# mehta-lab/VisCy

Hardware: AMD Instinct MI355X
Metric: training patches/sec (Z=5, 256x256, 1->2ch UNeXt2) (higher is better)
Workload: dtype bf16; 1 GPU; UNeXt2 2.5D convnextv2_tiny Z=5 256x256 1->2ch, fwd+MixedLoss(0.5,0,0.5)+bwd+AdamW; per_gpu_batch=512, global_batch=512, parallelism=dp1

## Files before the change

viscy_amd/csrc/gemm.hip:

```cpp
#include "vsx_common.h"
#include "mfma16.h"
#include "../../include/vsx.h"

bool vsx_gemm_nt2_ok(const VsxGemm* p);
bool vsx_gemm_nt2_lnbwd_ok(const VsxGemm* p);
void vsx_gemm_nt2_plan(const VsxGemm* p, VsxGemmPlan& pl);
int vsx_gemm_nt2_run(const VsxGemmPlan& pl, const VsxGemm* p, hipStream_t s);

struct RowCoord {
  int b, y, x;
  bool valid;
};

__device__ __forceinline__ RowCoord decode_row(const VsxGemm& p, int m) {
  RowCoord r;
  r.valid = m < p.M;
  int mm = r.valid ? m : 0;
  if (p.a_mode == VSX_A_ROWS && p.c_mode == VSX_A_ROWS) {
    r.b = p.hw > 0 ? mm / p.hw : 0;
    r.y = 0;
    r.x = mm;
  } else {
    int hw = p.gh * p.gw;
    r.b = mm / hw;
// ... 1092 lines not shown
#pragma unroll
    for (int i = 0; i < NCHX; ++i)
      if (livex[i]) xr[i] = ldvec_stream<T>(reinterpret_cast<const T*>(Xs + xoff[i]), x_once);
#pragma unroll
    for (int i = 0; i < NCHY; ++i)
      if (livey[i]) yr[i] = ldvec_stream<T>(reinterpret_cast<const T*>(Ys + yoff[i]), y_once);
  };
  float gsr[VN], gbr[VN];
  int gcur = -1;
  if constexpr (PRO == 1) {
#pragma unroll
    for (int j = 0; j < VN; ++j) gbr[j] = p.grn_b[kcol[0] + j];
  }
  auto store_tiles = [&](int step, int buf, const vec* xr, const vec* yr) {
    char* Xs = smem + buf * (TILE_X + TILE_Y);
    char* Ys = Xs + TILE_X;
    if constexpr (PRO == 1) {
      const int bnow = (step * BMS) / p.hw;
      if (bnow != gcur) {
        gcur = bnow;
        const float* gs = p.grn_s + (size_t)bnow * p.K + kcol[0];
#pragma unroll
        for (int j = 0; j < VN; ++j) gsr[j] = gs[j];
      }
    }
#pragma unroll
    for (int i = 0; i < NCHX; ++i) {
      if (livex[i]) {
        const vec xv = xr[i];
        *reinterpret_cast<vec*>(Xs + ldsx[i]) = xv;
      }
    }
#pragma unroll
    for (int i = 0; i < NCHY; ++i) {
      if (livey[i]) {
        vec yv = yr[i];
        if constexpr (PRO == 1) {
          float f[VN];
          unpack<T>(yv, f);
#pragma unroll
          for (int j = 0; j < VN; ++j) f[j] = fmaf(f[j], gsr[j], gbr[j]);
          yv = pack<T>(f);
        }
        *reinterpret_cast<vec*>(Ys + ldsy[i]) = yv;
      }
    }
  };

  mf_f32x4 acc[FN_][FK_];
  mfma_zero(acc);
  float csum = 0.f;
  const bool do_colsum = p.colsum != nullptr && tile_k == 0 && tid < BTN;
  mf_f32x4 acc2[PRO == 2 ? FN_ : 1][PRO == 2 ? FK_ : 1];
  float sreg[PRO == 2 ? FK_ : 1];
  mf_f32x4 acc1[2] = {{0.f, 0.f, 0.f, 0.f}, {0.f, 0.f, 0.f, 0.f}};
  frag_t ones_frag;
  const bool want_p = PRO == 2 && p.aux != nullptr && p.red0 != nullptr;
  if constexpr (PRO == 2) {
    union { unsigned short h[8]; frag_t v; } one;
#pragma unroll
    for (int j = 0; j < 8; ++j) one.h[j] = 0x3F80;
    ones_frag = one.v;
    mfma_zero(acc2);
    if (want_p) {
      const unsigned short* W2 = reinterpret_cast<const unsigned short*>(p.aux);
#pragma unroll
      for (int i = 0; i < FN_; ++i)
#pragma unroll
        for (int j = 0; j < FK_; ++j) {
          const int k = k0 + (wk * FK_ + j) * 16 + p16;
          unsigned short w[4];
#pragma unroll
          for (int r = 0; r < 4; ++r) {
            const int n = n0 + (wn * FN_ + i) * 16 + kq * 4 + r;
            w[r] = (n < p.N && k < p.K) ? W2[(size_t)n * p.ldx + k] : (unsigned short)0;
          }
          w2img[(i * FK_ + j) * 256 + tid] = make_uint2((uint32_t)w[0] | ((uint32_t)w[1] << 16), (uint32_t)w[2] | ((uint32_t)w[3] << 16));
        }
    }
  }

  const bool contig = (p.pro & 1024) != 0;
  const int sps = PRO == 2 ? p.hw / BMS : 1;
  const int units = total_steps / sps;
  const int sq = units / nsplit, sr = units % nsplit;
  const int sbase = (by * sq + (by < sr ? by : sr)) * sps;
  const int nsteps = contig ? (sq + (by < sr ? 1 : 0)) * sps : (total_steps - by + nsplit - 1) / nsplit;
  auto step_of = [&](int st) { return contig ? sbase + st : st * nsplit + by; };
  auto mma_step = [&](const char* Xs, const char* Ys) {
#pragma unroll
    for (int kk = 0; kk < BMS / MK; ++kk) {
      const char* Xk = Xs + (sizeof(T) == 2 ? kk * 32 * LDBX : 0);
      const char* Yk = Ys + (sizeof(T) == 2 ? kk * 32 * LDBY : 0);
      constexpr int JH = FK_ > 8 ? 2 : 1, JW = FK_ / JH;
      static_assert(FK_ % JH == 0, "Y fragments split evenly");
      frag_t xf[FN_], yf[JW];
#pragma unroll
      for (int i = 0; i < FN_; ++i) xf[i] = lds_frag_mn<T, TR>(Xk, LDBX, (wn * FN_ + i) * 16, p16, kq, kk);
#pragma unroll
      for (int jh = 0; jh < JH; ++jh) {
#pragma unroll
        for (int j = 0; j < JW; ++j) yf[j] = lds_frag_mn<T, TR>(Yk, LDBY, (wk * FK_ + jh * JW + j) * 16, p16, kq, kk);
#pragma unroll
        for (int i = 0; i < FN_; ++i)
#pragma unroll
          for (int j = 0; j < JW; ++j) acc[i][jh * JW + j] = mfma16(xf[i], yf[j], acc[i][jh * JW + j]);
      }
      if constexpr (PRO == 2) {
        static_assert(PRO != 2 || FN_ == 4, "two X fragments per wave");
#pragma unroll
        for (int h = 0; h < 2; ++h) acc1[h] = mfma16(wk == 0 ? xf[h] : xf[2 + h], ones_frag, acc1[h]);
      }
    }
    if constexpr (PRO == 2) {
    } else if (do_colsum) {
#pragma unroll 8
      for (int r = 0; r < BMS; ++r) csum += to_f32<T>(*reinterpret_cast<const T*>(Xs + r * LDBX + tid * ES));
    }
  };
  auto sample_begin = [&](int gstep) {
    if constexpr (PRO == 2) {
      const float* gs = p.grn_s + (size_t)(gstep / sps) * p.K;
#pragma unroll
      for (int j = 0; j < FK_; ++j) {
        const int k = k0 + (wk * FK_ + j) * 16 + p16;
        sreg[j] = gs[k < p.K ? k : p.K - 1];
      }
    }
  };
  auto sample_end = [&](int gstep) {
    if constexpr (PRO == 2) {
      if (want_p) {
        float pj[FK_];
#pragma unroll
        for (int j = 0; j < FK_; ++j) {
          float a = 0.f;
#pragma unroll
          for (int i = 0; i < FN_; ++i) {
            const uint2 w = w2img[(i * FK_ + j) * 256 + tid];
            a = fmaf(acc[i][j][0], __uint_as_float(w.x << 16), a);
            a = fmaf(acc[i][j][1], __uint_as_float(w.x & 0xFFFF0000u), a);
            a = fmaf(acc[i][j][2], __uint_as_float(w.y << 16), a);
            a = fmaf(acc[i][j][3], __uint_as_float(w.y & 0xFFFF0000u), a);
          }
          a += __shfl_xor(a, 16, 64);
          a += __shfl_xor(a, 32, 64);
          pj[j] = a;
        }
        if (kq == 0) {
          float* P = p.red0 + (size_t)(gstep / sps) * p.K;
#pragma unroll
          for (int j = 0; j < FK_; ++j) {
            const int k = k0 + (wk * FK_ + j) * 16 + p16;
            if (k < p.K) atomicAdd(P + k, pj[j]);
          }
        }
      }
#pragma unroll
      for (int i = 0; i < FN_; ++i)
#pragma unroll
        for (int j = 0; j < FK_; ++j)
#pragma unroll
          for (int r = 0; r < 4; ++r) {
            acc2[i][j][r] = fmaf(acc[i][j][r], sreg[j], acc2[i][j][r]);
            acc[i][j][r] = 0.f;
          }
    }
  };
  load_tiles(step_of(0), xreg, yreg);
  if constexpr (NBUF == 2) {
    store_tiles(step_of(0), 0, xreg, yreg);
    __syncthreads();
    for (int st = 0; st < nsteps; ++st) {
      const int nxt = step_of(st + 1);
      if (st + 1 < nsteps) load_tiles(nxt, xreg, yreg);
      const char* Xs = smem + (st & 1) * (TILE_X + TILE_Y);
      mma_step(Xs, Xs + TILE_X);
      if (st + 1 < nsteps) store_tiles(nxt, (st + 1) & 1, xreg, yreg);
      __syncthreads();
    }
  } else {
    static_assert(PRO != 2 || NBUF == 1, "the post-scaled weight gradient lives on the single-buffer geometry");
    for (int st = 0; st < nsteps; ++st) {
      store_tiles(step_of(st), 0, xreg, yreg);
      __syncthreads();
      if (st + 1 < nsteps) load_tiles(step_of(st + 1), xreg, yreg);
      if constexpr (PRO == 2) {
        if ((sbase + st) % sps == 0) sample_begin(sbase + st);
      }
      mma_step(smem, smem + TILE_X);
      if constexpr (PRO == 2) {
        if ((sbase + st + 1) % sps == 0) sample_end(sbase + st);
      }
      __syncthreads();
    }
  }
  if constexpr (PRO == 2) {
    float* cs = reinterpret_cast<float*>(smem);
    __syncthreads();
    if (p16 == 0) {
#pragma unroll
      for (int h = 0; h < 2; ++h)
#pragma unroll
        for (int r = 0; r < 4; ++r) cs[(wn * FN_ + 2 * wk + h) * 16 + kq * 4 + r] = acc1[h][r];
    }
    __syncthreads();
    if (tid < BTN) csum = cs[tid];
#pragma unroll
    for (int j = 0; j < FK_; ++j) {
      const int k = k0 + (wk * FK_ + j) * 16 + p16;
      const float bk = p.grn_b[k < p.K ? k : p.K - 1];
#pragma unroll
      for (int i = 0; i < FN_; ++i)
#pragma unroll
        for (int r = 0; r < 4; ++r) acc[i][j][r] = fmaf(bk, cs[(wn * FN_ + i) * 16 + kq * 4 + r], acc2[i][j][r]);
    }
  }

  const bool per_sample = p.b_bstride != 0;
  const bool ps_atomic = (p.pro & 4096) != 0;
  const int sample = per_sample ? (int)(((long)sbase * BMS) / p.hw) : 0;
  float* W = reinterpret_cast<float*>(p.C) + p.c_coff[z] + (per_sample ? (size_t)sample * (size_t)p.b_bstride : 0);
#pragma unroll
  for (int i = 0; i < FN_; ++i)
#pragma unroll
    for (int j = 0; j < FK_; ++j)
#pragma unroll
      for (int r = 0; r < 4; ++r) {
        const int n = n0 + (wn * FN_ + i) * 16 + kq * 4 + r;
        const int k = k0 + (wk * FK_ + j) * 16 + p16;
        if (n < p.N && k < p.K) {
          if (per_sample && !ps_atomic) W[(size_t)n * p.ldc + k] = acc[i][j][r];
          else atomicAdd(W + (size_t)n * p.ldc + k, acc[i][j][r]);
        }
      }
  if (do_colsum && n0 + tid < p.N) {
    if (per_sample && !ps_atomic) p.colsum[(size_t)sample * p.N + n0 + tid] = csum;
    else atomicAdd(p.colsum + (per_sample ? (size_t)sample * p.N : 0) + n0 + tid, csum);
  }
}

__global__ __launch_bounds__(256) void tn_zero_kernel(float* __restrict__ p, long n) {
  long i = ((long)blockIdx.x * 256 + threadIdx.x) * 4;
  if (i + 3 < n) *reinterpret_cast<float4*>(p + i) = make_float4(0.f, 0.f, 0.f, 0.f);
  else for (; i < n; ++i) p[i] = 0.f;
}

static double last_round_fill(long wgs, int per_cu) {
  const long slots = 256 * per_cu, rounds = (wgs + slots - 1) / slots;
  return (double)wgs / (double)(rounds * slots);
}

static int fill_splits(int tiles, int per_cu, int want, int max_splits) {
  if (!g_vsx_tn_fill) return want;
  int lo = want * 2 / 3, hi = want * 4 / 3;
  lo = lo < 1 ? 1 : lo;
  hi = hi > max_splits ? max_splits : hi;
  int best = want < lo ? lo : (want > hi ? hi : want);
  double best_fill = -1.0;
  for (int sp = lo; sp <= hi; ++sp) {
    const double fill = last_round_fill((long)tiles * sp, per_cu);
    const int d = sp > want ? sp - want : want - sp, bd = best > want ? best - want : want - best;
    if (fill > best_fill + 1e-9 || (fill > best_fill - 1e-9 && d < bd)) { best_fill = fill; best = sp; }
  }
  return best;
}

static int fill_sample_splits(int tiles, int per_cu, int ks, int steps) {
  if (!g_vsx_tn_fill) return ks;
  int best = ks;
  double best_fill = -1.0;
  for (int sp = ks; sp <= 4 * ks && sp <= 64 && steps % sp == 0; sp *= 2) {
    const double fill = last_round_fill((long)tiles * sp, per_cu);
    if (fill > best_fill + 1e-9) { best_fill = fill; best = sp; }
  }
  return best;
}

static int plan_tn(const VsxGemm* p, int dtype, VsxGemmPlan& pl) {
  if (int e = check_common(p, dtype, "vsx_gemm_tn")) return e;
  VSX_CHECK(p->epi == VSX_EPI_NONE && p->c_mode == VSX_A_ROWS, "vsx_gemm_tn: no epilogue / scatter modes");
  const long t128 = (long)vsx_cdiv(p->N, 128) * vsx_cdiv(p->K, 128);
  bool small = (p->N < 96 || p->K < 96) || (t128 < 24 && p->M < 65536);
  if (p->b_bstride != 0) small = false;
  const bool stats = p->pro == VSX_PRO_GRN && p->aux != nullptr && p->red0 != nullptr;
  if (stats) {
    VSX_CHECK(dtype == VSX_BF16 && g_vsx_tn_tr, "vsx_gemm_tn: the weight gradient with GRN statistics (aux = W2, red0 = P) is a bf16 kernel");
    small = false;
  }
  const int es = dtype == VSX_BF16 ? 2 : 4, vn = 16 / es, BT = small ? 64 : 128, nz = p->nz > 0 ? p->nz : 1;
  const bool TR = es == 2 && g_vsx_tn_tr, lean128 = TR && BT == 128;
  const unsigned long long ld_bytes = (unsigned long long)(p->lda > p->ldb ? p->lda : p->ldb) * es;
  const int stream_bits = (g_vsx_tn_stream & 3) << 13;
  pl = VsxGemmPlan{};
  pl.family = FAM_TN_FAST;
  pl.esize = es; pl.tr = TR; pl.tile[0] = pl.tile[1] = BT; pl.step = 32; pl.nbuf = 2; pl.block = 256;
  const int tiles = vsx_cdiv(p->N, BT) * vsx_cdiv(p->K, BT);
  const int want = vsx_cdiv(g_vsx_tn_want, tiles * nz), max_splits = vsx_cdiv(p->M, 256);
  int splits = want < 1 ? 1 : (want > max_splits ? max_splits : want);
  const int cap = tiles * nz <= 4 ? 384 : (tiles * nz <= 24 ? 96 : 48);
  if (splits > cap) splits = cap;
  if (splits > vsx_cdiv(p->M, 32)) splits = vsx_cdiv(p->M, 32);
  if (splits >= 8) splits &= ~7;
  pl.grid[0] = tiles; pl.grid[1] = splits; pl.grid[2] = nz;
  if (p->b_bstride != 0) {
    VSX_CHECK(lean128, "vsx_gemm_tn: per-sample outputs (b_bstride) exist for bf16 operands with outputs of at least 96 x 96 only");
    VSX_CHECK((g_vsx_nt_fast & 1) && p->a_mode == VSX_A_ROWS && p->pro == VSX_PRO_NONE && p->hw > 0 && p->hw % 64 == 0 && p->M % p->hw == 0 &&
                  nz == 1 && 64 * ld_bytes < (1ull << 31),
              "vsx_gemm_tn: per-sample outputs (b_bstride) need plain bf16 row operands, no prologue, hw %% 64 == 0");
    const int nb = p->M / p->hw;
    const bool n_full = p->N >= 192 && p->N <= 256 && p->K >= 128;
    const int t2 = n_full ? vsx_cdiv(p->N, 256) * vsx_cdiv(p->K, 128) : tiles;
    int ks = 1;
    const int spp = p->hw / 64;
    while ((long)nb * ks * t2 < 768 && ks < 64 && spp % (2 * ks) == 0) ks *= 2;
    if (ks > 1) ks = fill_sample_splits(nb * t2, n_full ? 2 : 3, ks, spp);
    pl.pro_bits = 1024 | stream_bits;
    if (ks > 1) {
      pl.pro_bits |= 4096;
      pl.zero_c = (long)nb * p->b_bstride;
      pl.zero_colsum = p->colsum ? (long)nb * p->N : 0;
    }
    if (n_full) { pl.tile[0] = 256; pl.tile[1] = 128; }
    pl.step = 64; pl.nbuf = 1;
    pl.grid[0] = t2; pl.grid[1] = nb * ks;
    return 0;
  }
  if (stats) {
    VSX_CHECK((g_vsx_nt_fast & 1) && p->a_mode == VSX_A_ROWS && nz == 1 && p->hw > 0 && p->hw % 64 == 0 && p->M % p->hw == 0 && p->N >= 96 &&
                  p->K >= 128 && p->N % 8 == 0 && p->K % 8 == 0 && p->ldx >= p->K && 64 * ld_bytes < (1ull << 31),
              "vsx_gemm_tn: the weight gradient with GRN statistics (aux = W2, red0 = P) needs plain bf16 row operands, hw %% 64 == 0, N >= 96, K >= 128");
    const int nb = p->M / p->hw;
    int sp = 1;
    if (g_vsx_tn_p2_rounds > 0) {
      sp = (g_vsx_tn_p2_rounds * 512) / tiles;
    } else {
      const int wantp = vsx_cdiv(g_vsx_tn_want * 2, tiles);
      for (int d = wantp < nb ? wantp : nb; d >= 1; --d)
        if (nb % d == 0) { sp = d; break; }
    }
    pl.pro_kind = 2; pl.step = 64; pl.nbuf = 1;
    pl.pro_bits = 1024 | stream_bits;
    pl.grid[1] = sp < 1 ? 1 : (sp > nb ? nb : sp);
    return 0;
  }
  const bool patch_ok = (g_vsx_nt_fast & 2) && p->a_mode == VSX_A_PATCH2 && p->pro == VSX_PRO_NONE && p->gw > 0 && (32 % p->gw == 0 || p->gw % 64 == 0) &&
                        p->cs % vn == 0 && (unsigned long long)(512 + 4 * p->gw) * p->lda * es < (1ull << 31);
  const bool fast = (g_vsx_nt_fast & 1) && (p->a_mode == VSX_A_ROWS || patch_ok) && p->M % 32 == 0 && p->N >= vn && p->K >= vn &&
                    (p->pro == VSX_PRO_NONE || (p->pro == VSX_PRO_GRN && p->hw > 0 && p->hw % 32 == 0)) && 32 * ld_bytes < (1ull << 31);
  if (!fast) {
    pl.family = FAM_TN_GEN;
    pl.step = pl.nbuf = 0;
    return 0;
  }
  pl.pro_kind = p->pro == VSX_PRO_GRN;
  pl.pro_bits = (g_vsx_tn_contig ? 1024 : 0) | stream_bits;
  if (!(es == 2 && BT == 128 && g_vsx_tn_wide && p->M % 64 == 0 && (p->pro == VSX_PRO_NONE || p->hw % 64 == 0) && p->M / 64 >= 2 * splits))
    return 0;
  pl.step = 64; pl.nbuf = 1;
  if (!TR) return 0;
  if (g_vsx_tn_fill) {
    int spf = fill_splits(tiles * nz, 3, splits, p->M / 128);
    if (spf > cap) spf = cap;
    pl.grid[1] = spf < 1 ? 1 : spf;
  }
  const bool n_div = (g_vsx_tn_rect & 2) && p->N % 256 == 0 && p->K >= 128 && p->pro == VSX_PRO_NONE;
  const bool n_full = ((g_vsx_tn_rect & 1) && p->N >= 224 && p->N <= 256 && p->K >= 256) || n_div;
  const bool k_full = (g_vsx_tn_rect & 1) && !n_full && p->K >= 224 && p->K <= 256 && p->N >= 256;
  if (!n_full && !k_full) return 0;
  pl.tile[0] = n_full ? 256 : 128; pl.tile[1] = n_full ? 128 : 256;
  const int t2 = vsx_cdiv(p->N, pl.tile[0]) * vsx_cdiv(p->K, pl.tile[1]);
  const int want2 = vsx_cdiv(g_vsx_tn_want2, t2 * nz);
  int sp2 = want2 < 1 ? 1 : (want2 > max_splits ? max_splits : want2);
  if (sp2 > p->M / 128) sp2 = p->M / 128;
  if (g_vsx_tn_fill) sp2 = fill_splits(t2 * nz, 2, sp2, p->M / 128);
  else if (sp2 >= 8) sp2 &= ~7;
  pl.grid[0] = t2; pl.grid[1] = sp2 < 1 ? 1 : sp2;
  return 0;
}

static int run_tn(const VsxGemmPlan& pl, const VsxGemm* p, hipStream_t s) {
  VsxGemm q = *p;
  q.pro = (pl.pro_kind == 2 ? 0 : q.pro) | pl.pro_bits;
  if (pl.zero_c) hipLaunchKernelGGL(tn_zero_kernel, dim3(vsx_cdiv(pl.zero_c, 1024L)), dim3(256), 0, s, reinterpret_cast<float*>(p->C) + p->c_coff[0], (long)pl.zero_c);
  if (pl.zero_colsum) hipLaunchKernelGGL(tn_zero_kernel, dim3(vsx_cdiv(pl.zero_colsum, 1024L)), dim3(256), 0, s, p->colsum, (long)pl.zero_colsum);
  const dim3 grid(pl.grid[0], pl.grid[1], pl.grid[2]), block(pl.block);
#define TN_GEN(T, BT, TR) \
  case inst_key(true, sizeof(T), BT, BT, 0, 0, 0, TR, 0): hipLaunchKernelGGL((gemm_tn_kernel<T, BT, TR>), grid, block, 0, s, q, 0); break;
#define TN_FAST1(T, BT, TR, PRO, BMS, NBUF, BTK) \
  case inst_key(false, sizeof(T), BT, BTK ? BTK : BT, BMS, NBUF, PRO, TR, 0): hipLaunchKernelGGL((gemm_tn_fast_kernel<T, BT, TR, PRO, BMS, NBUF, BTK>), grid, block, 0, s, q); break;
#define TN_FAST(T, BT, TR, BMS, NBUF, BTK)  TN_FAST1(T, BT, TR, 0, BMS, NBUF, BTK) TN_FAST1(T, BT, TR, 1, BMS, NBUF, BTK)
  switch (inst_key(pl)) {
    TN_GEN(bf16_t, 64, true) TN_GEN(bf16_t, 128, true) TN_GEN(bf16_t, 64, false) TN_GEN(bf16_t, 128, false) TN_GEN(float, 64, false) TN_GEN(float, 128, false)
    TN_FAST(bf16_t, 64, true, 32, 2, 0) TN_FAST(bf16_t, 128, true, 32, 2, 0)
    TN_FAST(bf16_t, 64, false, 32, 2, 0) TN_FAST(bf16_t, 128, false, 32, 2, 0)
    TN_FAST(float, 64, false, 32, 2, 0) TN_FAST(float, 128, false, 32, 2, 0)
    TN_FAST(bf16_t, 128, true, 64, 1, 0) TN_FAST(bf16_t, 128, false, 64, 1, 0)
    TN_FAST(bf16_t, 256, true, 64, 1, 128)
    TN_FAST(bf16_t, 128, true, 64, 1, 256)
    TN_FAST1(bf16_t, 128, true, 2, 64, 1, 0)
    default: vsx_set_error("vsx_gemm_tn: the plan names no instantiation"); return 1;
  }
#undef TN_GEN
#undef TN_FAST1
#undef TN_FAST
  VSX_LAUNCH_CHECK();
  g_vsx_last_kernel = pl.family;
  return 0;
}

extern "C" int32_t vsx_gemm_tn(const VsxGemm* p, int32_t dtype, vsx_stream_t stream) {
  VsxGemmPlan pl;
  if (int e = plan_tn(p, dtype, pl)) return e;
  return run_tn(pl, p, reinterpret_cast<hipStream_t>(stream));
}

extern "C" int32_t vsx_gemm_plan(int32_t kind, const VsxGemm* p, int32_t dtype, VsxGemmPlan* out) {
  VSX_CHECK(out != nullptr && (kind == VSX_GEMM_NT || kind == VSX_GEMM_TN), "vsx_gemm_plan: kind %d, out %p", kind, (void*)out);
  return kind == VSX_GEMM_NT ? plan_nt(p, dtype, *out) : plan_tn(p, dtype, *out);
}
```

viscy_amd/engine_unext2.py:

```python

from __future__ import annotations

import os
from collections import namedtuple
from typing import NamedTuple

import torch
from torch import Tensor

from . import _lib as L
from . import ops as hip_ops
from .flat import FlatEngine, engine_apply


class _BlockW:

    __slots__ = ("C", "p", "dw_w", "W1f", "W1fT", "b1f", "W2", "W2T", "v1", "fc2_w", "fc2_b", "grn_w", "grn_b", "dp", "img", "img2", "b2f")


class _ProjW:
    __slots__ = ("cin", "cout", "taps", "ln", "conv", "W", "WT")


FWD_UNFUSED, FWD_PAIR, FWD_FC1 = 0, 1, 2


class _MlpPlan(NamedTuple):

    fwd: int
    ln_in: bool
    keep_h: bool
    keep_xh: bool
    bwd: int
    tn_stats: bool


def _plan_mlp(flag: int, supported, C: int, hw: int, M: int, B: int, dt: torch.dtype, training: bool, ln_bwd_ok: bool,
              tn_stats_ok: bool) -> _MlpPlan:
    if dt != torch.bfloat16:
        flag = 0
    if not training:
        pair = bool(flag & 1) and supported(None)
        return _MlpPlan(FWD_PAIR if pair else FWD_UNFUSED, pair and bool(flag & 32), False, False, 0, False)
    fc1 = bool(flag & 2) and supported(2)
    bwd = 0
    if flag & 8 and supported(4):
        if B * C * 4 * C * 4 <= (512 << 20) and C >= 96 and hw % 64 == 0:
            bwd = 1
        elif supported(3):
            bwd = 2
    recompute_h = bool(flag & 64) and bwd != 0 and supported(5) and supported(6)
    drop_xh = bool(flag & 128) and bool(flag & 32) and recompute_h and supported(7) and ln_bwd_ok
    ln_in = fc1 and bool(flag & 32)
    return _MlpPlan(FWD_FC1 if fc1 else FWD_UNFUSED, ln_in, not (fc1 and recompute_h), not (ln_in and drop_xh), bwd,
                    bwd == 2 and bool(tn_stats_ok))


_BlockSaved = namedtuple("_BlockSaved", "x xh rstd h gact colsq s rows dpm plan y mean")
_NarrowSaved = namedtuple("_NarrowSaved", "x y colsq s")


def _views(flat: Tensor, shapes):
    out, off = [], 0
    for shp in shapes:
        n = 1
        for s in shp:
            n *= s
        out.append(flat[off : off + n].view(shp))
        off += n
    return out


class _ZeroArena:

    def __init__(self, dev, numel: int, ops):
        self.dev, self.ops = dev, ops
        self.buf = self._zeros(numel) if numel > 0 else None
        self.off = 0
        self.used = 0

    def _zeros(self, *shape) -> Tensor:
        return self.ops.zeros(*shape, device=self.dev)

    def take(self, *shape) -> Tensor:
        n = 1
        for d in shape:
            n *= int(d)
        n_al = (n + 63) // 64 * 64
        self.used += n_al
        if self.buf is not None and self.off + n_al <= self.buf.numel():
            v = self.buf[self.off:self.off + n].view(*shape)
            self.off += n_al
            return v
        return self._zeros(*shape)


class Engine(FlatEngine):
    name = "UNeXt2"

    def __init__(self, model, ops=None):
        ops = hip_ops if ops is None else ops
        self._hip = ops is hip_ops
        self._mlp_flag = 0
        self.cfg = model.cfg
        self._zeros4c = {}
        self._dp_inject = None
        self._za = None
        self._za_need = {}
        self._prepared_for = None
        self.W = None
        super().__init__(model, ops)

    def _stage_params_rev(self, stage):
        ps = []
        for blk in reversed(list(stage.blocks)):
            if hasattr(blk, "gamma"):
                ps += [blk.gamma, blk.mlp.fc2.weight, blk.mlp.fc2.bias, blk.mlp.fc1.weight, blk.mlp.fc1.bias, blk.norm.weight,
                       blk.norm.bias, blk.conv_dw.weight, blk.conv_dw.bias]
                continue
            ps += [blk.mlp.fc2.weight, blk.mlp.fc2.bias, blk.mlp.grn.weight, blk.mlp.grn.bias, blk.mlp.fc1.weight,
                   blk.mlp.fc1.bias, blk.norm.weight, blk.norm.bias, blk.conv_dw.weight, blk.conv_dw.bias]
        if not isinstance(stage.downsample, torch.nn.Identity):
            ps += [stage.downsample[1].weight, stage.downsample[1].bias, stage.downsample[0].weight,
                   stage.downsample[0].bias]
        return ps

    def _param_order(self):
        m = self.model
        ps = []
        if self.cfg.get("head", "conv") == "conv":
# ... 100 lines not shown
        narrow_stem = cfg.get("head") == "shuffle" and tuple(cfg["stem_kernel"][1:]) == (2, 2)
        if narrow_stem and K % 8 and Dp == 1:
            W["stem_W"], W["stem_b"] = None, m.stem.conv.bias
        elif Dp == 1:
            W["stem_W"], _ = o.prep_weight(sw, co3, K, 1, dt)
            if dt == torch.bfloat16 and K % 32:
                o.flush()
                W["stem_W"] = o.pad_cols(W["stem_W"], (K + 31) // 32 * 32)
            W["stem_b"] = m.stem.conv.bias
        else:
            we = torch.zeros((co3, Dp, Dp, K), dtype=torch.float32, device=self.device)
            for d in range(Dp):
                we[:, d, d, :] = sw.detach().reshape(co3, K)
            W["stem_W"] = we.reshape(co3 * Dp, Dp * K).to(dt).contiguous()
            W["stem_b"] = m.stem.conv.bias.detach().repeat_interleave(Dp).contiguous()
        s2 = getattr(m, "stem2d", None)
        if s2 is not None:
            K2 = s2.weight[0].numel()
            W["stem2d_W"] = None
            if not (narrow_stem and K2 % 8):
                W["stem2d_W"], _ = o.prep_weight(s2.weight, s2.weight.shape[0], K2, 1, dt)
            if W["stem2d_W"] is not None and dt == torch.bfloat16 and K2 % 32:
                o.flush()
                W["stem2d_W"] = o.pad_cols(W["stem2d_W"], (K2 + 31) // 32 * 32)
            W["stem2d_b"] = s2.bias
        enc = []
        for i in range(4):
            st = getattr(m.encoder_stages, f"stages_{i}")
            proj = None
            if not isinstance(st.downsample, torch.nn.Identity):
                proj = self._prep_proj(st.downsample[0], st.downsample[1], dt, need_bwd)
            enc.append((proj, [self._prep_block(b, dt, need_bwd) for b in st.blocks]))
        rates = cfg.get("drop_path")
        if rates:
            flat_blocks = [bw for _, blocks in enc for bw in blocks]
            assert len(rates) == len(flat_blocks)
            for bw, r in zip(flat_blocks, rates):
                bw.dp = float(r)
        W["enc"] = enc
        dec = []
        if cfg.get("head") == "embed":
            t = m.tail
            E, Cf = t.fc0.weight.shape
            P = t.fc3.weight.shape[0]
            W["fc0"], W["fc0T"] = o.prep_weight(t.fc0.weight, E, Cf, 1, torch.float32, want=True, want_t=need_bwd)
            W["fc3"], W["fc3T"] = o.prep_weight(t.fc3.weight, P, E, 1, torch.float32, want=True, want_t=need_bwd)
        else:
            for us in m.decoder.decoder_stages:
                st = us.conv
                proj = self._prep_proj(st.downsample[0], st.downsample[1], dt, need_bwd)
                dec.append((proj, [self._prep_block(b, dt, need_bwd) for b in st.blocks]))
            pre = []
            for us in m.decoder.decoder_stages:
                pc = getattr(us, "pre_conv", None)
                if pc is None:
                    pre.append(None)
                else:
                    cpc = pc.weight.shape[0]
                    pre.append((pc, *o.prep_weight(pc.weight, cpc, cpc, 9, dt, want=True, want_t=need_bwd)))
            W["dec_pre"] = pre
        W["dec"] = dec
        if cfg.get("head", "conv") == "conv":
            hc = m.head.conv[0].conv
            cmid, c3 = hc.weight.shape[0], hc.weight.shape[1]
            hdt = self._head_dtype(dt)
            W["head_Wc"], _ = o.prep_weight(hc.weight, cmid, c3, 27, hdt, tapmode=1)
            if need_bwd:
                if hdt == torch.bfloat16 and c3 == 8 and cmid == 32 and cfg["out_stack_depth"] == 5:
                    o.flush()
                    W["head_Wp"] = o.head_conv_dgrad_prep(W["head_Wc"])
                W["head_Wd"] = o.prep_head_dgrad(hc.weight, cmid, c3, cfg["out_stack_depth"], hdt)
        return W

    def _head_dtype(self, dt: torch.dtype) -> torch.dtype:
        if dt == torch.bfloat16 and self.model.head.conv[0].conv.weight.shape[1] % 8:
            return torch.float32
        return dt

    def _plan(self, C, hw, M, B, dt, training: bool) -> _MlpPlan:
        o, flag = self.ops, self._mlp_flag
        ask = training and dt == torch.bfloat16 and flag != 0
        return _plan_mlp(flag, lambda mode: o.mlp_supported(C, hw, M, dt, mode), C, hw, M, B, dt, training,
                         ask and bool(L.lib().vsx_gemm_nt_ln_bwd_supported(M, C, 4 * C, L.dtype_code(dt))),
                         ask and o.tn_grn_stats_ok(M, C, 4 * C, hw, dt))

    def _block_fwd(self, x, w, B, H, Wd, dt, save, rows=None):
        if w.C < 16:
            return self._block_fwd_narrow(x, w, B, H, Wd, save, rows)
        o = self.ops
        C, M = w.C, B * H * Wd
        blk = w.p
        hw = H * Wd
        y = o.dwconv7_fwd(x, w.dw_w, blk.conv_dw.bias, B, H, Wd, C)
        xres = x
        if rows is not None:
            idx, inv, _, Lr = rows
            M, hw = B * Lr, Lr
            y = o.rows_select(y, idx, M, C)
            xres = o.rows_select(x, idx, M, C)
        plan = self._plan(C, hw, M, B, dt, save is not None)
        mean = rstd = None
        if plan.ln_in:
            xh = None
        else:
            xh, _, rstd = o.ln_fwd(y, None, None, M, C, 1e-6, need_mean=False)
            y = None
        colsq = self._za.take(B, 4 * C)
        dpm = None
        if w.dp > 0.0 and self.model.training:
            inj = self._dp_inject
            dpm = inj.pop(0) if inj else (torch.rand(B, device=x.device) < (1.0 - w.dp)).float() / (1.0 - w.dp)
        assert plan.fwd == FWD_UNFUSED or w.img is not None
        if plan.fwd == FWD_PAIR:
            src, lne = (y, 1e-6) if plan.ln_in else (xh, 0.0)
            o.mlp_stats(src, w.img, w.b1f, colsq, M, C, hw, ln_eps=lne)
            s = o.grn_scale(colsq, w.grn_w)
            out = o.mlp_out(src, w.img, w.b1f, s, w.grn_b, w.fc2_b, xres, dpm, M, C, hw, ln_eps=lne)
            if rows is not None:
                out = o.rows_select(out, rows[1], B * H * Wd, C)
            return out
        if plan.fwd == FWD_FC1:
            if plan.ln_in:
                first, rstd, h, gact = o.mlp_fc1_ln(y, w.img, w.b1f, colsq, M, C, hw, 1e-6, store_h=plan.keep_h,
                                                    store_xh=plan.keep_xh)
                xh, y, mean = (first, None, None) if plan.keep_xh else (None, *first)
                del first
            else:
                h, gact = o.mlp_fc1(xh, w.img, w.b1f, colsq, M, C, hw, store_h=plan.keep_h)
        else:
            h = torch.empty((M, 4 * C), dtype=dt, device=x.device) if save is not None else None
            gact = torch.empty((M, 4 * C), dtype=dt, device=x.device)
            o.gemm("nt", xh, w.W1f, h, M, 4 * C, C, C, C, 4 * C, dtype=dt, epi=L.EPI_BIAS_GELU_SQ, bias=w.b1f, red0=colsq,
                   hw=hw, C2=gact)
        s = o.grn_scale(colsq, w.grn_w)
        out = torch.empty((M, C), dtype=dt, device=x.device)
        if dt == torch.bfloat16 and C > 64 and hw % 128 == 0 and hw // 128 >= 8:
            Ws = o.scale_weight_samples(w.fc2_w, s, dt)
            b2 = w.b2f
            if b2 is None:
                b2 = o.matvec(w.fc2_w, w.grn_b, w.fc2_b, C, 4 * C)
                o.flush()
            o.gemm("nt", gact, Ws, out, M, C, 4 * C, 4 * C, 4 * C, C, dtype=dt, hw=hw, b_bstride=C * 4 * C,
                   epi=L.EPI_BIAS_RES, bias=b2, res=xres, ldr=C, rscale=dpm)
        else:
            o.gemm("nt", gact, w.W2, out, M, C, 4 * C, 4 * C, 4 * C, C, dtype=dt, pro=L.PRO_GRN, grn_s=s,
                   grn_b=w.grn_b, hw=hw, epi=L.EPI_BIAS_RES, bias=w.fc2_b, res=xres, ldr=C, rscale=dpm)
        if rows is not None:
            out = o.rows_select(out, rows[1], B * H * Wd, C)
        if save is not None:
            save.append(_BlockSaved(x, xh, rstd, h, gact, colsq, s, rows, dpm, plan, y, mean))
        return out

    def _block_fwd_narrow(self, x, w, B, H, Wd, save, rows):
        o, C = self.ops, w.C
        if rows is not None or w.v1 or (w.dp > 0.0 and self.model.training):
            raise NotImplementedError("narrow ConvNeXt blocks are built for dense ConvNeXt-V2 decoder stages only")
        colsq = self._za.take(B, 4 * C)
        y = o.narrow_block_fwd1(x, w.dw_w, w.p.conv_dw.bias, w.W1f, w.b1f, colsq, B, H, Wd, C)
        s = o.grn_scale(colsq, w.grn_w)
        out = o.narrow_block_fwd2(y, x, w.W1f, w.b1f, s, w.grn_b, w.W2, w.fc2_b, B, H, Wd, C)
        if save is not None:
            save.append(_NarrowSaved(x, y, colsq, s))
        return out

    def _block_bwd_narrow(self, dout, w, saved, B, H, Wd):
        o, g = self.ops, self.g
        C, blk = w.C, w.p
# ... 485 lines not shown
```

viscy_amd/ops.py:

```python

from __future__ import annotations

import contextlib
import ctypes as C
import os
import threading
from typing import Sequence

import torch
from torch import Tensor

from . import _lib as L
from ._lib import VsxGemm, VsxGemmPlan, check, dtype_code, lib, ptr, stream


class Scratch:

    def __init__(self, alloc=None):
        self._alloc = alloc or (lambda floats, dev: torch.empty(floats, dtype=torch.float32, device=dev))
        self._tls = threading.local()
        self.held: list = []

    def take(self, dev, floats: int):
        arenas = getattr(self._tls, "arenas", None)
# ... 39 lines not shown
        for i, v in enumerate(vals):
            arr[i] = int(v)


def gemm(
    kind: str,
    A: Tensor,
    B: Tensor,
    Cout: Tensor,
    M: int,
    N: int,
    K: int,
    lda: int,
    ldb: int,
    ldc: int,
    *,
    dtype: torch.dtype,
    a_mode: int = L.A_ROWS,
    gh: int = 0,
    gw: int = 0,
    cs: int = 0,
    nz: int = 1,
    a_coff: Sequence[int] | None = None,
    b_off: Sequence[int] | None = None,
    c_coff: Sequence[int] | None = None,
    c_mode: int = L.A_ROWS,
    c_cs: int = 0,
    pro: int = L.PRO_NONE,
    grn_s: Tensor | None = None,
    grn_b: Tensor | None = None,
    hw: int = 0,
    epi: int = L.EPI_NONE,
    bias: Tensor | None = None,
    res: Tensor | None = None,
    ldr: int = 0,
    aux: Tensor | None = None,
    ldx: int = 0,
    red0: Tensor | None = None,
    red1: Tensor | None = None,
    colsum: Tensor | None = None,
    C2: Tensor | None = None,
    b_bstride: int = 0,
    rscale: Tensor | None = None,
    plan: VsxGemmPlan | None = None,
) -> None:
    for t in (bias, grn_s, grn_b, red0, red1, colsum):
        if t is not None and t.dtype != torch.float32:
            raise TypeError("bias / GRN / reduction buffers must be float32")
    p = VsxGemm()
    p.A, p.B, p.C = ptr(A), ptr(B), ptr(Cout)
    p.M, p.N, p.K = M, N, K
    p.lda, p.ldb, p.ldc = lda, ldb, ldc
    p.a_mode, p.gh, p.gw, p.cs = a_mode, gh, gw, cs
    p.nz = nz
    _fill8(p.a_coff, a_coff)
    _fill8(p.b_off, b_off)
    _fill8(p.c_coff, c_coff)
    p.c_mode, p.c_cs = c_mode, c_cs
    p.pro = pro
    p.grn_s, p.grn_b = ptr(grn_s), ptr(grn_b)
    p.hw = hw
    p.epi = epi
    p.bias, p.res, p.ldr = ptr(bias), ptr(res), ldr
    p.aux, p.ldx = ptr(aux), ldx
    p.red0, p.red1, p.colsum = ptr(red0), ptr(red1), ptr(colsum)
    p.C2 = ptr(C2)
    p.b_bstride = b_bstride
    p.rscale = ptr(rscale)
    if plan is not None:
        return check(lib().vsx_gemm_plan(L.GEMM_NT if kind == "nt" else L.GEMM_TN, C.byref(p), dtype_code(dtype), C.byref(plan)), f"gemm_plan_{kind}")
    if kind == "nt" and epi == L.EPI_BIAS_GELU_SQ:
        _det(A.device, lambda: _gemm_det_floats(p, dtype))
    fn = lib().vsx_gemm_nt if kind == "nt" else lib().vsx_gemm_tn
    check(fn(C.byref(p), dtype_code(dtype), stream()), f"gemm_{kind}")


def _gemm_det_floats(p: VsxGemm, dtype: torch.dtype) -> int:
    plan = VsxGemmPlan()
    check(lib().vsx_gemm_plan(L.GEMM_NT, C.byref(p), dtype_code(dtype), C.byref(plan)), "gemm_plan_nt")
    return plan.det_floats


def tn_grn_stats_ok(M: int, N: int, K: int, hw: int, dtype: torch.dtype) -> bool:
    if dtype != torch.bfloat16 or not lib().vsx_get_flag(b"tn_rect") & 8:
        return False
    p = VsxGemm()
    p.A = p.B = p.C = p.grn_s = p.grn_b = p.aux = p.red0 = 1
    p.M, p.N, p.K, p.lda, p.ldb, p.ldc, p.ldx, p.nz, p.pro, p.hw = M, N, K, K, N, K, K, 1, L.PRO_GRN, hw
    return lib().vsx_gemm_plan(L.GEMM_TN, C.byref(p), L.VSX_BF16, C.byref(VsxGemmPlan())) == 0


def dgrad_ln_bwd(dh: Tensor, WT: Tensor, xh: Tensor, rstd: Tensor, M: int, C: int, K: int,
                 mean: Tensor | None = None) -> Tensor | None:
    if dh.dtype != torch.bfloat16 or not lib().vsx_gemm_nt_ln_bwd_supported(M, C, K, dtype_code(dh.dtype)):
        return None
    dy = torch.empty((M, C), dtype=dh.dtype, device=dh.device)
    gemm("nt", dh, WT, dy, M, C, K, K, K, C, dtype=dh.dtype, epi=L.EPI_LN_BWD, aux=xh, ldx=C, grn_s=rstd, grn_b=mean)
    return dy


def gemm_z(kind: str, *args, nz: int, a_coff, b_off, c_coff, **kw) -> None:
    for s in range(0, nz, 8):
        e = min(nz, s + 8)
        gemm(kind, *args, nz=e - s, a_coff=a_coff[s:e], b_off=b_off[s:e], c_coff=c_coff[s:e], **kw)


def ln_fwd(x: Tensor, gamma: Tensor | None, beta: Tensor | None, rows: int, Cc: int, eps: float = 1e-6,
           need_mean: bool = True):
    y = torch.empty_like(x)
    mean = torch.empty(rows, dtype=torch.float32, device=x.device) if need_mean else None
    rstd = torch.empty(rows, dtype=torch.float32, device=x.device)
    check(lib().vsx_ln_fwd(ptr(x), ptr(y), ptr(mean), ptr(rstd), ptr(gamma), ptr(beta), rows, Cc, eps,
                           dtype_code(x.dtype), stream()), "ln_fwd")
    return y, mean, rstd


def ln_bwd(dy: Tensor, x: Tensor, mean: Tensor | None, rstd: Tensor, gamma: Tensor | None, add: Tensor | None,
           dgamma: Tensor | None, dbeta: Tensor | None, rows: int, Cc: int) -> Tensor:
    dx = torch.empty_like(dy)
    check(lib().vsx_ln_bwd(ptr(dy), ptr(x), ptr(mean), ptr(rstd), ptr(gamma), ptr(add), ptr(dx), ptr(dgamma),
                           ptr(dbeta), rows, Cc, dtype_code(dy.dtype), stream()), "ln_bwd")
    return dx


def grn_scale(colsq: Tensor, gamma: Tensor, eps: float = 1e-6) -> Tensor:
    s = torch.empty_like(colsq)
    check(lib().vsx_grn_scale(ptr(colsq), ptr(gamma), ptr(s), colsq.shape[0], colsq.shape[1], eps, stream()), "grn_scale")
    return s


def grn_bwd_stats(colsq: Tensor, P: Tensor, gamma: Tensor, dgamma: Tensor, eps: float = 1e-6, Sb: Tensor | None = None,
                  dbeta: Tensor | None = None) -> Tensor:
    t = torch.empty_like(colsq)
    rowst = torch.empty_like(colsq)
    if _BATCH is not None:
        nb, N = colsq.shape
        check(lib().vsx_grn_bwd_stats(ptr(colsq), ptr(P), None, ptr(gamma), ptr(t), None, None, ptr(rowst), nb, N, eps, stream()),
              "grn_bwd_stats")
        _queue(L.WTASK_REDUCE_ROWS, 0, (nb, N), rowst, dgamma, None, None)
        if Sb is not None:
            _queue(L.WTASK_REDUCE_ROWS, 0, (nb, N), Sb, dbeta, None, None)
        return t
    check(lib().vsx_grn_bwd_stats(ptr(colsq), ptr(P), ptr(Sb), ptr(gamma), ptr(t), ptr(dgamma), ptr(dbeta), ptr(rowst), colsq.shape[0],
                                  colsq.shape[1], eps, stream()), "grn_bwd_stats")
    return t


def grn_gelu_bwd(dz: Tensor, h: Tensor, s: Tensor, t: Tensor, colsum: Tensor, M: int, N: int, hw: int) -> None:
    rows = 2048
    ws = _workspace(dz.device, rows * N)
    check(lib().vsx_grn_gelu_bwd(ptr(dz), ptr(h), ptr(s), ptr(t), ptr(colsum), ptr(ws), rows, M, N, hw,
                                 dtype_code(dz.dtype), stream()), "grn_gelu_bwd")


def dwconv7_fwd(x: Tensor, w: Tensor, bias: Tensor | None, B: int, H: int, W: int, Cc: int) -> Tensor:
    y = torch.empty_like(x)
    check(lib().vsx_dwconv7_fwd(ptr(x), ptr(w), ptr(bias), None, ptr(y), B, H, W, Cc, dtype_code(x.dtype), stream()),
          "dwconv7_fwd")
    return y


def dwconv7_bwd_data(dy: Tensor, w: Tensor, add: Tensor | None, B: int, H: int, W: int, Cc: int) -> Tensor:
    dx = torch.empty_like(dy)
    check(lib().vsx_dwconv7_bwd_data(ptr(dy), ptr(w), ptr(add), ptr(dx), B, H, W, Cc, dtype_code(dy.dtype), stream()),
          "dwconv7_bwd_data")
    return dx


def dwconv7_bwd_weight(dy: Tensor, x: Tensor, dw: Tensor, db: Tensor | None, B: int, H: int, W: int, Cc: int) -> None:
    rows = 256
    ws = _workspace(dy.device, rows * 50 * Cc)
    check(lib().vsx_dwconv7_bwd_weight(ptr(dy), ptr(x), ptr(dw), ptr(db), ptr(ws), rows, B, H, W, Cc, dtype_code(dy.dtype),
# ... 1184 lines not shown
```

Measured before the change: 5637 patches/s.

## Allow sub-sample step splits in GRN-stats weight-gradient GEMM and prefer it when grid fills

The GRN-statistics weight-gradient kernel can now split work at step granularity instead of whole-sample units when there are too few samples per split, with partial samples accumulating their P contributions through the existing atomics. The planner accepts a negative rounds flag that sets the split count directly, above the sample count. The MLP planner selects the fused stats backward (bwd=2) for C<=192 when the resulting grid has at least 384 blocks. The P dot product also accumulates in a 4-wide vector FMA. This trades more atomic traffic for better GPU occupancy on narrow stages.

```diff
diff --git a/viscy_amd/csrc/gemm.hip b/viscy_amd/csrc/gemm.hip
--- a/viscy_amd/csrc/gemm.hip
+++ b/viscy_amd/csrc/gemm.hip
@@ -1198,10 +1198,11 @@
 
   const bool contig = (p.pro & 1024) != 0;
   const int sps = PRO == 2 ? p.hw / BMS : 1;
-  const int units = total_steps / sps;
+  const int unit = total_steps / sps >= 8 * nsplit ? sps : 1;
+  const int units = total_steps / unit;
   const int sq = units / nsplit, sr = units % nsplit;
-  const int sbase = (by * sq + (by < sr ? by : sr)) * sps;
-  const int nsteps = contig ? (sq + (by < sr ? 1 : 0)) * sps : (total_steps - by + nsplit - 1) / nsplit;
+  const int sbase = (by * sq + (by < sr ? by : sr)) * unit;
+  const int nsteps = contig ? (sq + (by < sr ? 1 : 0)) * unit : (total_steps - by + nsplit - 1) / nsplit;
   auto step_of = [&](int st) { return contig ? sbase + st : st * nsplit + by; };
   auto mma_step = [&](const char* Xs, const char* Ys) {
 #pragma unroll
@@ -1250,15 +1251,15 @@
         float pj[FK_];
 #pragma unroll
         for (int j = 0; j < FK_; ++j) {
-          float a = 0.f;
+          mf_f32x4 a4 = {0.f, 0.f, 0.f, 0.f};
 #pragma unroll
           for (int i = 0; i < FN_; ++i) {
             const uint2 w = w2img[(i * FK_ + j) * 256 + tid];
-            a = fmaf(acc[i][j][0], __uint_as_float(w.x << 16), a);
-            a = fmaf(acc[i][j][1], __uint_as_float(w.x & 0xFFFF0000u), a);
-            a = fmaf(acc[i][j][2], __uint_as_float(w.y << 16), a);
-            a = fmaf(acc[i][j][3], __uint_as_float(w.y & 0xFFFF0000u), a);
+            const mf_f32x4 wf = {__uint_as_float(w.x << 16), __uint_as_float(w.x & 0xFFFF0000u), __uint_as_float(w.y << 16),
+                                 __uint_as_float(w.y & 0xFFFF0000u)};
+            a4 = __builtin_elementwise_fma(acc[i][j], wf, a4);
           }
+          float a = (a4[0] + a4[1]) + (a4[2] + a4[3]);
           a += __shfl_xor(a, 16, 64);
           a += __shfl_xor(a, 32, 64);
           pj[j] = a;
@@ -1302,11 +1303,11 @@
       __syncthreads();
       if (st + 1 < nsteps) load_tiles(step_of(st + 1), xreg, yreg);
       if constexpr (PRO == 2) {
-        if ((sbase + st) % sps == 0) sample_begin(sbase + st);
+        if (st == 0 || (sbase + st) % sps == 0) sample_begin(sbase + st);
       }
       mma_step(smem, smem + TILE_X);
       if constexpr (PRO == 2) {
-        if ((sbase + st + 1) % sps == 0) sample_end(sbase + st);
+        if (st + 1 == nsteps || (sbase + st + 1) % sps == 0) sample_end(sbase + st);
       }
       __syncthreads();
     }
@@ -1447,8 +1448,11 @@
                   p->K >= 128 && p->N % 8 == 0 && p->K % 8 == 0 && p->ldx >= p->K && 64 * ld_bytes < (1ull << 31),
               "vsx_gemm_tn: the weight gradient with GRN statistics (aux = W2, red0 = P) needs plain bf16 row operands, hw %% 64 == 0, N >= 96, K >= 128");
     const int nb = p->M / p->hw;
-    int sp = 1;
-    if (g_vsx_tn_p2_rounds > 0) {
+    int sp = 1, max_sp = nb;
+    if (g_vsx_tn_p2_rounds < 0) {
+      sp = -g_vsx_tn_p2_rounds;
+      max_sp = p->M / 64 < 65535 ? p->M / 64 : 65535;
+    } else if (g_vsx_tn_p2_rounds > 0) {
       sp = (g_vsx_tn_p2_rounds * 512) / tiles;
     } else {
       const int wantp = vsx_cdiv(g_vsx_tn_want * 2, tiles);
@@ -1457,7 +1461,7 @@
     }
     pl.pro_kind = 2; pl.step = 64; pl.nbuf = 1;
     pl.pro_bits = 1024 | stream_bits;
-    pl.grid[1] = sp < 1 ? 1 : (sp > nb ? nb : sp);
+    pl.grid[1] = sp < 1 ? 1 : (sp > max_sp ? max_sp : sp);
     return 0;
   }
   const bool patch_ok = (g_vsx_nt_fast & 2) && p->a_mode == VSX_A_PATCH2 && p->pro == VSX_PRO_NONE && p->gw > 0 && (32 % p->gw == 0 || p->gw % 64 == 0) &&
diff --git a/viscy_amd/engine_unext2.py b/viscy_amd/engine_unext2.py
--- a/viscy_amd/engine_unext2.py
+++ b/viscy_amd/engine_unext2.py
@@ -23,6 +23,7 @@
 
 
 FWD_UNFUSED, FWD_PAIR, FWD_FC1 = 0, 1, 2
+TN_STATS_MAX_C = 192
 
 
 class _MlpPlan(NamedTuple):
@@ -36,7 +37,7 @@
 
 
 def _plan_mlp(flag: int, supported, C: int, hw: int, M: int, B: int, dt: torch.dtype, training: bool, ln_bwd_ok: bool,
-              tn_stats_ok: bool) -> _MlpPlan:
+              tn_stats_ok: bool, tn_stats_fills: bool = False) -> _MlpPlan:
     if dt != torch.bfloat16:
         flag = 0
     if not training:
@@ -45,7 +46,9 @@
     fc1 = bool(flag & 2) and supported(2)
     bwd = 0
     if flag & 8 and supported(4):
-        if B * C * 4 * C * 4 <= (512 << 20) and C >= 96 and hw % 64 == 0:
+        if tn_stats_ok and tn_stats_fills and C <= TN_STATS_MAX_C:
+            bwd = 2
+        elif B * C * 4 * C * 4 <= (512 << 20) and C >= 96 and hw % 64 == 0:
             bwd = 1
         elif supported(3):
             bwd = 2
@@ -312,7 +315,7 @@
         ask = training and dt == torch.bfloat16 and flag != 0
         return _plan_mlp(flag, lambda mode: o.mlp_supported(C, hw, M, dt, mode), C, hw, M, B, dt, training,
                          ask and bool(L.lib().vsx_gemm_nt_ln_bwd_supported(M, C, 4 * C, L.dtype_code(dt))),
-                         ask and o.tn_grn_stats_ok(M, C, 4 * C, hw, dt))
+                         ask and o.tn_grn_stats_ok(M, C, 4 * C, hw, dt), ask and o.tn_grn_stats_fills(M, C, 4 * C, hw, dt))
 
     def _block_fwd(self, x, w, B, H, Wd, dt, save, rows=None):
         if w.C < 16:
diff --git a/viscy_amd/ops.py b/viscy_amd/ops.py
--- a/viscy_amd/ops.py
+++ b/viscy_amd/ops.py
@@ -145,12 +145,22 @@
 
 
 def tn_grn_stats_ok(M: int, N: int, K: int, hw: int, dtype: torch.dtype) -> bool:
+    return _tn_grn_stats_plan(M, N, K, hw, dtype) is not None
+
+
+def _tn_grn_stats_plan(M: int, N: int, K: int, hw: int, dtype: torch.dtype) -> VsxGemmPlan | None:
     if dtype != torch.bfloat16 or not lib().vsx_get_flag(b"tn_rect") & 8:
-        return False
+        return None
     p = VsxGemm()
     p.A = p.B = p.C = p.grn_s = p.grn_b = p.aux = p.red0 = 1
     p.M, p.N, p.K, p.lda, p.ldb, p.ldc, p.ldx, p.nz, p.pro, p.hw = M, N, K, K, N, K, K, 1, L.PRO_GRN, hw
-    return lib().vsx_gemm_plan(L.GEMM_TN, C.byref(p), L.VSX_BF16, C.byref(VsxGemmPlan())) == 0
+    plan = VsxGemmPlan()
+    return plan if lib().vsx_gemm_plan(L.GEMM_TN, C.byref(p), L.VSX_BF16, C.byref(plan)) == 0 else None
+
+
+def tn_grn_stats_fills(M: int, N: int, K: int, hw: int, dtype: torch.dtype) -> bool:
+    plan = _tn_grn_stats_plan(M, N, K, hw, dtype)
+    return plan is not None and plan.grid[0] * plan.grid[1] >= 384
 
 
 def dgrad_ln_bwd(dh: Tensor, WT: Tensor, xh: Tensor, rstd: Tensor, M: int, C: int, K: int,
```

After: 5662 patches/s (median of 2 runs). About the same (+0.4%).
